# nlesc-smcm/hymls

Hardware: AMD Instinct MI355X
Metric: Preconditioner ApplyInverse DoF/s + achieved HBM GB/s, Stokes3D (higher is better)
Workload: dtype f64

## Files before the change

hymls_amd/api.py:

```python
import ctypes as C
import os
import numpy as np

LIB_PATH = os.environ.get("HYMLS_MI_LIBRARY") or os.path.join(os.path.dirname(os.path.abspath(__file__)), "libhymls_mi.so")


class HymlsError(RuntimeError):
    def __init__(self, code, msg):
        super().__init__("hymls_mi error %d: %s" % (code, msg))
        self.code = code


class _Params(C.Structure):
    _fields_ = [(n, C.c_int32) for n in (
        "nx", "ny", "nz", "dim", "equations", "dof", "sx", "sy", "sz", "cx", "cy", "cz", "levels",
        "partitioner", "retain_nodes", "retain_pressures", "link_velocities", "link_retained",
        "fix_pressure_level", "nfix")] + [("fix_gid", C.c_int32 * 4), ("variable_type", C.c_int32 * 8),
                                         ("retain_xyz", C.c_int32 * 3), ("retain_at_level", C.c_int32 * 8),
                                         ("retain_at_level_xyz", (C.c_int32 * 3) * 8), ("periodic", C.c_int32 * 3)]


_I32P = C.POINTER(C.c_int32)
_I64P = C.POINTER(C.c_int64)
_F64P = C.POINTER(C.c_double)
# ... 26 lines not shown
        "hymls_mi_default_params": (None, [C.POINTER(_Params)]),
        "hymls_mi_create": (C.c_int, [C.POINTER(H), C.POINTER(_Params), C.c_int]),
        "hymls_mi_set_matrix_csr": (C.c_int, [H, C.c_int64, _I32P, _I32P, _F64P]),
        "hymls_mi_set_comm": (C.c_int, [H, C.POINTER(_Comm), C.c_int, C.c_int, C.c_int]),
        "hymls_mi_rank_grid": (C.c_int, [C.c_int, C.POINTER(C.c_int), C.POINTER(C.c_int), C.POINTER(C.c_int)]),
        "hymls_mi_device_alloc": (C.c_void_p, [H, C.c_int64]),
        "hymls_mi_device_free": (None, [H, C.c_void_p]),
        "hymls_mi_copy_to_host": (C.c_int, [H, C.c_void_p, C.c_void_p, C.c_int64]),
        "hymls_mi_copy_to_device": (C.c_int, [H, C.c_void_p, C.c_void_p, C.c_int64]),
        "hymls_mi_rccl_unique_id": (C.c_int, [C.c_char_p]),
        "hymls_mi_rccl_comm_init": (C.c_int, [C.c_char_p, C.c_int, C.c_int, C.c_int, C.POINTER(C.c_void_p)]),
        "hymls_mi_rccl_comm_destroy": (None, [C.c_void_p]),
        "hymls_mi_set_comm_rccl": (C.c_int, [H, C.c_void_p, C.c_int, C.c_int, C.c_int]),
        "hymls_mi_comm_selftest": (C.c_int, [H]),
        "hymls_mi_invert_blocks": (C.c_int, [H, C.c_int32, C.c_int32, _F64P]),
        "hymls_mi_required_rows": (C.c_int, [H, _I64P, _I32P]),
        "hymls_mi_set_matrix_rows": (C.c_int, [H, C.c_int64, _I32P, _I32P, _I32P, _F64P]),
        "hymls_mi_owned_rows": (C.c_int, [H, _I64P, _I32P]),
        "hymls_mi_generate_rows": (C.c_int, [C.c_int, C.c_int, C.c_int, C.c_int, C.c_double, C.c_double, C.c_int64, _I32P,
                                             _I64P, _I32P, _I32P, _F64P]),
        "hymls_mi_set_testvector": (C.c_int, [H, _F64P]),
        "hymls_mi_initialize": (C.c_int, [H]),
        "hymls_mi_compute": (C.c_int, [H]),
        "hymls_mi_set_factor_storage": (C.c_int, [H, C.c_int]),
        "hymls_mi_factor_storage": (C.c_int, [H]),
        "hymls_mi_apply_inverse": (C.c_int, [H, C.c_void_p, C.c_int64, C.c_void_p, C.c_int64, C.c_int, C.c_int]),
        "hymls_mi_set_border": (C.c_int, [H, C.c_int, C.c_void_p, C.c_int64, C.c_void_p, C.c_int64, C.c_void_p]),
        "hymls_mi_apply_inverse_bordered": (C.c_int, [H, C.c_void_p, C.c_void_p, C.c_void_p, C.c_void_p, C.c_int]),
        "hymls_mi_apply": (C.c_int, [H, _F64P, _F64P]),
        "hymls_mi_matvec": (C.c_int, [H, C.c_void_p, C.c_void_p, C.c_int]),
# ... 165 lines not shown
            self.SetFactorStorage(storage)
        if comm is not None:
            comm.attach(self)
            px, py, pz = rank_grid
            if getattr(comm, "nccl_comm", None) is not None:
                self._check(self._lib.hymls_mi_set_comm_rccl(self._h, comm.nccl_comm, px, py, pz))
            else:
                self._check(self._lib.hymls_mi_set_comm(self._h, C.byref(comm.c_struct), px, py, pz))
        if K is not None:
            self.SetMatrix(K)
        if testVector is not None:
            self.SetTestVector(testVector)

    def CommSelfTest(self):
        return self._lib.hymls_mi_comm_selftest(self._h)

    def InvertBlocks(self, blocks):
        B = np.asarray(blocks, dtype=np.float64)
        assert B.ndim == 3 and B.shape[1] == B.shape[2]
        cm = np.array(B.transpose(0, 2, 1), dtype=np.float64, order="C", copy=True)
        self._check(self._lib.hymls_mi_invert_blocks(self._h, B.shape[1], B.shape[0], cm.ctypes.data_as(_F64P)))
        return np.ascontiguousarray(cm.transpose(0, 2, 1))

    def RequiredRows(self):
        n = C.c_int64()
        self._check(self._lib.hymls_mi_required_rows(self._h, C.byref(n), None))
        g = np.empty(n.value, np.int32)
        self._check(self._lib.hymls_mi_required_rows(self._h, C.byref(n), _i32(g)))
        return g

# ... 264 lines not shown
```

hymls_amd/csrc/capi.cpp:

```cpp
#include "../../include/hymls_mi.h"
#include "precond.hpp"
#include "capi_internal.hpp"
#include <chrono>
#include <cstring>

namespace hymls {
int64_t generate_laplace3d(int nx, int ny, int nz, int32_t* rowptr, int32_t* col, double* val);
int64_t generate_stokes3d(int nx, int ny, int nz, double a, double b, int32_t* rowptr, int32_t* col, double* val);
int64_t generate_rows(int equations, int nx, int ny, int nz, double a, double b, int64_t nrows, const int32_t* gids,
                      int32_t* rowptr, int32_t* col, double* val, double re, const bool* per);
}

using namespace hymls;

struct hymls_mi {
  Params p;
  int device = 0;
  dev::Context* ctx = nullptr;
  Csr K;
  bool have_matrix = false;
  Comm comm;
  ivec gids;
  int32_t nrows = 0;
  ivec rows_rowptr, rows_colgid;
// ... 231 lines not shown
    int32_t* d_flag = (int32_t*)dev::alloc(sizeof(int32_t));
    int32_t flag = 0;
    try {
      dev::h2d(d, blocks, bytes);
      dev::zero(d_flag, sizeof(int32_t));
      dev::dense_invert(nb, nblk, d, d_flag);
      dev::d2h(&flag, d_flag, sizeof flag);
      dev::d2h(blocks, d, bytes);
    } catch (...) { dev::free(d); dev::free(d_flag); throw; }
    dev::free(d); dev::free(d_flag);
    HYMLS_CHECK(flag == 0, -4, "singular block");
  }
  API_END(h)
}

int hymls_mi_required_rows(hymls_mi_t* h, int64_t* n, int32_t* gids) {
  if (!h || !n) return -2;
  API_BEGIN
  if (!h->top) { h->top.reset(new LevelSolver(h->p, 0, h->ngid(), &h->comm)); h->initialized = false; h->n_init_top = 0; }
  h->top->partition(nullptr);
  ivec r = h->top->required_gids();
  *n = (int64_t)r.size();
  if (gids) std::copy(r.begin(), r.end(), gids);
  API_END(h)
}

int hymls_mi_set_matrix_rows(hymls_mi_t* h, int64_t nrows, const int32_t* gids, const int32_t* rowptr,
                             const int32_t* colgid, const double* val) {
  if (!h || !gids || !rowptr) return -2;
  API_BEGIN
// ... 408 lines not shown
```

hymls_amd/csrc/device.hpp:

```cpp
#pragma once
#include <cstdio>
#include "common.hpp"
#include "symbolic.hpp"

namespace hymls {
namespace dev {

struct Context;
Context* create_context(int device);
void bind(Context* c);
Context* current();
void destroy_context(Context* c);
void* stream();
const double* zeros16();
void* alloc(size_t bytes);
void free(void* p);
void h2d(void* dst, const void* src, size_t bytes);
void d2h(void* dst, const void* src, size_t bytes);
void d2d(void* dst, const void* src, size_t bytes);
void zero(void* dst, size_t bytes);
void sync();
size_t mem_free();
void* shared_scratch(size_t bytes);
constexpr int NSIDE = 8;
// ... 76 lines not shown
  double* swork;
  int64_t swork_stride;
};

void gather(int64_t n, const int32_t* idx, const double* src, double* dst);
void scatter(int64_t n, const int32_t* idx, const double* src, double* dst);
void scatter_add(int64_t n, const int32_t* idx, const double* src, double* dst);
void axpby(int64_t n, double a, const double* x, double b, double* y);
void scale_copy(int64_t n, double a, const double* x, double* y);
inline int spmv_lanes(int32_t nrows, int64_t nnz_hint) {
  const double avg = nnz_hint >= 0 ? (double)nnz_hint / nrows : 8.0;
  return avg < 2.5 ? 1 : (avg < 5.0 ? 2 : (avg < 20.0 ? 4 : 8));
}
void spmv(int32_t nrows, const int32_t* rowptr, const int32_t* col, const double* val,
          const double* x, double* y, double alpha, double beta, int64_t nnz_hint = -1);
void pull_sum(int64_t n, const int64_t* ptr, const int64_t* idx, const double* in, double* out);
void offdiag_count(int64_t nrows, const int32_t* rows, const int32_t* krow, const int32_t* kcol, const int32_t* ta, const int32_t* tb,
                   const int32_t* excl, int32_t* count);
void offdiag_fill(int64_t nrows, const int32_t* rows, const int32_t* krow, const int32_t* kcol, const int32_t* ta, const int32_t* tb,
                  const int32_t* excl, const int32_t* rowptr, int32_t* col, int32_t* src);
void member_sources(int32_t nb, int32_t next, int32_t nent, const int32_t* ext, const int32_t* ent_row, const int32_t* ent_col,
                    const int32_t* krow, const int32_t* kcol, int32_t* src, int32_t* flag);
void build_pull_tables(int64_t nrows, const int64_t* rcount, const int32_t* rowptr, const uint64_t* keys, int64_t* ptr, int64_t* idx);
void pull_sum_blocks(int64_t blen, int32_t nblk, const int64_t* ptr, const int64_t* base,
                     const double* in, double* out);

void factor_level(const PlanD& P, const BatchD& B, const int32_t* list, int32_t count,
                  int32_t b0, int32_t nbc, const double* kval, int32_t max_w);
void sblock_init(const PlanD& P, const BatchD& B, int32_t b0, int32_t nbc, const double* kval);

// ... 55 lines not shown
                     const double* x, double* y);
void solve_bwd_tasks(const LvlTask* tasks, int32_t ntasks, const LvlSub* subs, const PlanD* plans, int32_t lds_doubles,
                     const double* y, double* x);

constexpr int NV_MAX = 4;
void interior_solve_fused_mv(int32_t nsub, const FusedSub* subs, const PlanD* plans, int32_t lds_doubles, int32_t front_doubles,
                             double* x, int64_t ldx, int nv);
void interior_solve_fused_mv_f32(int32_t nsub, const FusedSub* subs, const PlanD* plans, int32_t lds_doubles, int32_t front_doubles,
                                 double* x, int64_t ldx, int nv);
void solve_fwd_tasks_mv(const LvlTask* tasks, int32_t ntasks, const LvlSub* subs, const PlanD* plans, int32_t lds_doubles,
                        const double* x, double* y, int64_t ld, int nv);
void solve_bwd_tasks_mv(const LvlTask* tasks, int32_t ntasks, const LvlSub* subs, const PlanD* plans, int32_t lds_doubles,
                        const double* y, double* x, int64_t ld, int nv);

void ot_apply(int32_t ng, const int32_t* gptr, const double* w, double* x);
void sblock_transform(int32_t nS, int32_t ng, const int32_t* gptr, const double* tv,
                      double* sblock, int32_t nbc);
void sblock_extract(int32_t nS, int64_t npick, const int32_t* pick, const double* sblock,
                    double* out, int64_t out_stride, int32_t nbc);
struct KeptD {
  int32_t nS, ngl;
  const int32_t* gptr; const int32_t* glink; const int32_t* goff; const int64_t* lboff; const int32_t* lblen;
};
void sblock_kept(const KeptD& K, const double* tv, const double* sblock, double* out, int64_t out_stride, int32_t nbc);
bool sblock_kept_fits(int32_t nS, int32_t ngl);
void dense_invert(int32_t nb, int32_t nblk, double* blocks, int32_t* flag);
bool dense_invert_blocked_order(int32_t nb);
void blocks_apply(int32_t nb, int32_t nblk, const double* binv, const int32_t* ids,
                  const double* x, double* y);

// ... 11 lines not shown
```

hymls_amd/csrc/device_hip.hip:

```cpp
#include <hip/hip_runtime.h>
#include <type_traits>
#include <dlfcn.h>
#include <chrono>
#include <cstring>
#include <cfloat>
#include <array>
#include <map>
#include <string>
#include <cstdio>
#include "device.hpp"

namespace hymls {
namespace dev {

#define HIP_CHECK(call)                                                                    \
  do {                                                                                     \
    hipError_t e_ = (call);                                                                \
    if (e_ != hipSuccess)                                                                  \
      throw ::hymls::Error(-3, std::string("HIP error: ") + hipGetErrorString(e_) + " at " + \
                                   __FILE__ + ":" + std::to_string(__LINE__));             \
  } while (0)

struct MarkRec { int phase; bool begin; hipEvent_t ev; };
struct Context {
// ... 260 lines not shown
  for (int64_t i = blockIdx.x * (int64_t)blockDim.x + threadIdx.x; i < n; i += (int64_t)gridDim.x * blockDim.x) atomicAdd(&dst[idx[i]], src[i]);
}
void scatter_add(int64_t n, const int32_t* idx, const double* src, double* dst) {
  if (n <= 0) return;
  hipLaunchKernelGGL(k_scatter_add, dim3(nblocks(n, 256, 65536)), dim3(256), 0, g_stream, n, idx, src, dst); launch_check();
}
void axpby(int64_t n, double a, const double* x, double b, double* y) {
  if (n <= 0) return;
  hipLaunchKernelGGL(k_axpby, dim3(nblocks(n, 256, 8192)), dim3(256), 0, g_stream, n, a, x, b, y); launch_check();
}
void scale_copy(int64_t n, double a, const double* x, double* y) {
  if (n <= 0) return;
  hipLaunchKernelGGL(k_scale_copy, dim3(nblocks(n, 256, 8192)), dim3(256), 0, g_stream, n, a, x, y); launch_check();
}

template <int L>
__global__ void k_spmv(int32_t nrows, const int32_t* __restrict__ rp, const int32_t* __restrict__ col,
                       const double* __restrict__ val, const double* __restrict__ x, double* __restrict__ y,
                       double alpha, double beta) {
  const int lane = (int)(threadIdx.x % L);
  const int rpb = (int)blockDim.x / L;
  for (int64_t base = (int64_t)blockIdx.x * rpb; base < nrows; base += (int64_t)gridDim.x * rpb) {
    const int64_t row = base + threadIdx.x / L;
    double s = 0.0;
    if (row < nrows) {
      const int b = rp[row], e = rp[row + 1];
      for (int k = b + lane; k < e; k += L) s += val[k] * x[col[k]];
    }
#pragma unroll
    for (int off = L / 2; off > 0; off >>= 1) s += __shfl_down(s, off, L);
    if (row < nrows && lane == 0) y[row] = alpha * s + (beta == 0.0 ? 0.0 : beta * y[row]);
  }
}
void spmv(int32_t nrows, const int32_t* rp, const int32_t* col, const double* val, const double* x, double* y,
          double alpha, double beta, int64_t nnz_hint) {
  if (nrows <= 0) return;
  const int L = spmv_lanes(nrows, nnz_hint);
  const int64_t nt = (int64_t)nrows * L;
  const dim3 grid(nblocks(nt, 256));
  switch (L) {
    case 1: hipLaunchKernelGGL(k_spmv<1>, grid, dim3(256), 0, g_stream, nrows, rp, col, val, x, y, alpha, beta); break;
    case 2: hipLaunchKernelGGL(k_spmv<2>, grid, dim3(256), 0, g_stream, nrows, rp, col, val, x, y, alpha, beta); break;
    case 4: hipLaunchKernelGGL(k_spmv<4>, grid, dim3(256), 0, g_stream, nrows, rp, col, val, x, y, alpha, beta); break;
    default: hipLaunchKernelGGL(k_spmv<8>, grid, dim3(256), 0, g_stream, nrows, rp, col, val, x, y, alpha, beta); break;
  }
  launch_check();
}

__global__ void k_pull_sum(int64_t n, const int64_t* __restrict__ ptr, const int64_t* __restrict__ idx,
                           const double* __restrict__ in, double* __restrict__ out) {
  for (int64_t e = blockIdx.x * (int64_t)blockDim.x + threadIdx.x; e < n; e += (int64_t)gridDim.x * blockDim.x) {
    double s = 0.0;
    for (int64_t t = ptr[e]; t < ptr[e + 1]; t++) s += in[idx[t]];
    out[e] = s;
  }
}
void pull_sum(int64_t n, const int64_t* ptr, const int64_t* idx, const double* in, double* out) {
  if (n <= 0) return;
  hipLaunchKernelGGL(k_pull_sum, dim3(nblocks(n, 256, 65536)), dim3(256), 0, g_stream, n, ptr, idx, in, out); launch_check();
// ... 1654 lines not shown

struct FusedFront { int32_t c0, w, ri, c_off, a_off, lf_off, idx_off, pad; int64_t lp_off, q_off; };
template <class PTR>
__device__ inline PTR lside(PTR base, int packed, int r, int w, int ri, int& c1, int& tri) {
  if (!packed) { c1 = w + ri; tri = 0; return base + r; }
  if (r < w) { c1 = w; tri = 1; return base + (r - 1); }
  c1 = ri; tri = 0;
  return base + ((w * (w - 1)) >> 1) + (r - w);
}
template <class PTR>
__device__ inline PTR uside(PTR base, int packed, int i, int w, int ri, int& c1, int& tri) {
  if (!packed) { c1 = w + ri; tri = 0; return base + i; }
  c1 = 0; tri = 1;
  return base + ((w * (w - 1)) >> 1) + ri * w + i;
}
template <int L>
__device__ __forceinline__ void fused_spmv_rows(int n, int tid, gptr<int32_t> rp, gptr<int32_t> col, gptr<double> val, gptr<double> x, double* y) {
  const int lane = tid % L, rpb = 256 / L;
  for (int base = 0; base < n; base += rpb) {
    const int row = base + tid / L;
    double s = 0.0;
    if (row < n) {
      const int b = rp[row], e = rp[row + 1];
      for (int k = b + lane; k < e; k += L) s += val[k] * x[col[k]];
    }
#pragma unroll
    for (int off = L / 2; off > 0; off >>= 1) s += __shfl_down(s, off, L);
    if (row < n && lane == 0) y[row] = s + 0.0;
  }
}
template <bool PROF, class PT, int IN, int OUT>
__device__ __forceinline__ void interior_fused_body(const FusedSub* __restrict__ subs, const PlanD* __restrict__ plans,
                                                    double* __restrict__ x, long long* __restrict__ prof, const FusedIO io) {
  extern __shared__ double lds[];
  auto ldp = [](gptr<PT> q) { return (double)*q; };
  long long tp[6] = {0, 0, 0, 0, 0, 0}, t0 = 0, tstart = 0;
  auto tick = [&](int bucket) { if (PROF) { const long long t = wall_clock64(); tp[bucket] += t - t0; t0 = t; } };
  if (PROF) { t0 = wall_clock64(); tstart = t0; }
  const FusedSub S = subs[blockIdx.x];
  const PlanD P = plans[S.cls];
  double* X = lds;
  double* C = lds + P.nI;
  double* Fv = C + P.contrib_size;
// ... 808 lines not shown
    else if (!fwd) solve_bwd_tasks(tasks, ntasks, subs, plans, lds_doubles, av, bv);
    else if (v == 0) solve_fwd_tasks(tasks, ntasks, subs, plans, lds_doubles, av, bv);
    else launch_lvl_mv<1>(fwd, tasks, ntasks, subs, plans, lds_doubles, av, bv, ld, v);
    v += g;
  }
}
void solve_fwd_tasks_mv(const LvlTask* tasks, int32_t ntasks, const LvlSub* subs, const PlanD* plans, int32_t lds_doubles,
                        const double* x, double* y, int64_t ld, int nv) {
  lvl_tasks_mv(true, tasks, ntasks, subs, plans, lds_doubles, x, y, ld, nv);
}
void solve_bwd_tasks_mv(const LvlTask* tasks, int32_t ntasks, const LvlSub* subs, const PlanD* plans, int32_t lds_doubles,
                        const double* y, double* x, int64_t ld, int nv) {
  lvl_tasks_mv(false, tasks, ntasks, subs, plans, lds_doubles, y, x, ld, nv);
}

__global__ void __launch_bounds__(256) k_ot(int32_t ng, const int32_t* __restrict__ gptr, const double* __restrict__ w, double* __restrict__ x) {
  const int g = blockIdx.x * 32 + (threadIdx.x >> 3);
  const int lane = threadIdx.x & 7;
  const bool on = g < ng;
  const int b = on ? gptr[g] : 0, e = on ? gptr[g + 1] : 0;
  double s = 0.0;
  for (int i = b + lane; i < e; i += 8) s += w[i] * x[i];
#pragma unroll
  for (int off = 4; off > 0; off >>= 1) s += __shfl_xor(s, off, 64);
  for (int i = b + lane; i < e; i += 8) x[i] = 2.0 * w[i] * s - x[i];
}
void ot_apply(int32_t ng, const int32_t* gptr, const double* w, double* x) {
  if (ng <= 0) return;
  hipLaunchKernelGGL(k_ot, dim3((ng + 31) / 32), dim3(256), 0, g_stream, ng, gptr, w, x); launch_check();
}

__device__ inline bool hh_setup(const double* v, int n, double& sg, double& nrm, double& v1, double& fac1) {
  sg = v[0] < 0 ? -1.0 : (v[0] > 0 ? 1.0 : 0.0);
  double s = 0.0;
  for (int i = 0; i < n; i++) s += v[i] * v[i];
  nrm = sqrt(s) * fabs(sg);
  v1 = sg * v[0] + nrm;
  if (fabs(v1) < 1e-14 || nrm < 1e-14) return false;
  fac1 = 1.0 / (nrm * v1);
  return true;
}
template <int PASS>
__global__ void __launch_bounds__(256) k_sblock_hh(int32_t nS, int32_t ng, const int32_t* __restrict__ gptr,
                                                    const double* __restrict__ tv, double* __restrict__ sblock) {
// ... 633 lines not shown
```

hymls_amd/csrc/precond.cpp:

```cpp
#include "precond.hpp"
#include <cstring>
#include <chrono>
#include <thread>
#include <mutex>
#include <atomic>
#include <map>
#include <unordered_map>

namespace hymls {

namespace {

struct Hasher {
  uint64_t h = 1469598103934665603ULL;
  void add(const void* p, size_t n) {
    const unsigned char* c = (const unsigned char*)p;
    size_t i = 0;
    for (; i + 8 <= n; i += 8) {
      uint64_t w;
      std::memcpy(&w, c + i, 8);
      h = (h ^ w) * 0x9E3779B97F4A7C15ULL;
      h ^= h >> 29;
    }
    for (; i < n; i++) { h ^= c[i]; h *= 1099511628211ULL; }
// ... 953 lines not shown
  d_t2_ = (double*)dev::alloc((size_t)std::max(n2_ + ngs_, 1) * sizeof(double));
  d_y2_ = (double*)dev::alloc((size_t)std::max(n2_, 1) * sizeof(double));
  d_yb_ = (double*)dev::alloc((size_t)std::max(n2_, 1) * sizeof(double));
  d_a12_val_ = (double*)dev::alloc(std::max<size_t>(1, a12_col_.size()) * sizeof(double));
  d_a21_val_ = (double*)dev::alloc(std::max<size_t>(1, a21_col_.size()) * sizeof(double));
  d_flag_ = (int32_t*)dev::alloc(sizeof(int32_t));
  {
    int64_t covered = 0;
    for (size_t c = 0; c < cls_.size(); c++)
      if (cls_fused_[c]) covered += (int64_t)cls_[c]->lu.plan.nI * (int64_t)cls_[c]->lu.members.size();
    fused_io_ = n1_ > 0 && covered == n1_ && merged_.nsubs == 0 && !std::getenv("HYMLS_MI_NO_FUSED_IO");
    if (std::getenv("HYMLS_MI_VERBOSE"))
      std::fprintf(stderr, "[hymls_mi] rank %d level %d: vector passes of the apply %s the interior solve (fused classes cover %lld of %d interior rows, A12 %.2f entries per row)\n",
                   comm_->rank, level_, fused_io_ ? "fused into" : "separate from", (long long)covered, n1_, n1_ ? (double)a12_col_.size() / n1_ : 0.0);
  }
  initialized_ = true;
}

void LevelSolver::build_classes() {
  const bool verbose_bc = std::getenv("HYMLS_MI_VERBOSE") != nullptr && (level_ == 0 || std::atoi(std::getenv("HYMLS_MI_VERBOSE")) >= 2);
  double t_bc = wall();
  auto lap_bc = [&](const char* what) {
    if (!verbose_bc) return;
    std::fprintf(stderr, "[hymls_mi] rank %d level %d:   classes / %-22s %.2f s\n", comm_->rank, level_, what, wall() - t_bc);
    t_bc = wall();
  };
  const int n = K_.n;
  const int nsd = (int)hm_.sd.size();
  const int nsep = n2_ + ngs_;
  auto sidx = [&](int32_t gid) { const int l = g2l_[gid]; return l >= 0 ? pos2_[l] : -1; };
// ... 1169 lines not shown

void LevelSolver::next_apply(const double* rhs, double* sol, int64_t ld, int nv) {
  if (!comm_->distributed()) { next_->apply_inverse_mv(rhs, ld, sol, ld, nv); return; }
  const int64_t ldn = std::max<int64_t>(n_next_owned_, 1);
  for (int v = 0; v < nv; v++) xch_down_.forward(rhs + v * ld, d_nrhs_ + v * ldn);
  next_->apply_inverse_mv(d_nrhs_, ldn, d_nsol_, ldn, nv);
  for (int v = 0; v < nv; v++) {
    if (next_is_direct_) {
      if (red_.n) dev::d2d(sol + v * ld, d_nsol_ + v * ldn + glob_row_off_[comm_->rank], (size_t)red_.n * sizeof(double));
    } else {
      xch_down_.backward(d_nsol_ + v * ldn, sol + v * ld);
    }
  }
}

void LevelSolver::schur_apply(double* rhs2, int64_t ldr, double* x2, int64_t ldx, int nv) {
  dev::Range range("SchurPreconditioner", level_ + 1, "ApplyInverse");
  if (global_n2_ == 0) return;
  if (direct_schur_) {
    if (!comm_->distributed()) { next_->apply_inverse_mv(rhs2, ldr, x2, ldx, nv); return; }
    for (int v = 0; v < nv; v++) next_apply(rhs2 + v * ldr, x2 + v * ldx, 0, 1);
    return;
  }
  const int ng = (int)vs_.size();
  const int64_t ldv = std::max(ng, 1);
  for (int v = 0; v < nv; v++) dev::ot_apply(ng, d_gptr_, d_otw_, rhs2 + v * ldr);
  dev::blocks_apply_all_mv(n_blk_apply_, d_blka_, blk_max_nb_, rhs2, ldr, x2, ldx, nv);
  for (int v = 0; v < nv; v++) dev::gather(ng, d_vs_, rhs2 + v * ldr, d_vrhs_ + v * ldv);
  if (profiling && level_ == 0) dev::mark(4, true);
  next_apply(d_vrhs_, d_vsol_, ldv, nv);
  if (profiling && level_ == 0) dev::mark(4, false);
  for (int v = 0; v < nv; v++) {
    dev::scatter(ng, d_vs_, d_vsol_ + v * ldv, x2 + v * ldx);
    dev::ot_apply(ng, d_gptr_, d_otw_, x2 + v * ldx);
  }
}

void LevelSolver::apply_inverse(const double* b, double* x) { apply_inverse_mv(b, 0, x, 0, 1); }

void LevelSolver::apply_inverse_mv(const double* b, int64_t ldb, double* x, int64_t ldx, int nv) {
  dev::Range range("Preconditioner", level_ + 1, "ApplyInverse");
  HYMLS_CHECK(next_ != nullptr || global_n2_ == 0, -1, "The preconditioner has not yet been computed.");
  ensure_nvec(nv);
  const int64_t ldz = n1_ + ngi_ + n2_, ld1 = std::max(n1_, 1), ld2 = std::max(n2_ + ngs_, 1);
  double* z1 = d_z_;
  double* z2 = d_z_ + n1_ + ngi_;
  const bool fio = fused_io_ && nv == 1;
  if (profiling) dev::mark(0, true);
  for (int v = 0; v < nv; v++) {
    if (!fio) dev::gather(n1_, d_inperm_, b + v * ldb, z1 + v * ldz);
    dev::gather(n2_, d_inperm_ + n1_, b + v * ldb, z2 + v * ldz);
  }
  if (profiling) dev::mark(1, true);
  if (fio) {
    dev::FusedIO io;
    io.in = 1; io.b = b; io.perm = d_inperm_;
    interior_solve_mv(z1, ldz, 1, &io);
  } else {
    interior_solve_mv(z1, ldz, nv);
  }
  if (profiling) { dev::mark(1, false); dev::mark(2, true); }
  for (int v = 0; v < nv; v++) {
    xch_int_.forward(z1 + v * ldz, z1 + v * ldz);
    dev::spmv(n2_, d_a21_row_, d_a21_col_, d_a21_val_, z1 + v * ldz, z2 + v * ldz, -1.0, 1.0, (int64_t)a21_col_.size());
  }
  if (profiling) { dev::mark(2, false); dev::mark(3, true); }
  schur_apply(z2, ldz, d_t2_, ld2, nv);
  if (profiling) dev::mark(3, false);
  if (fio) {
    xch_sep_.forward(d_t2_, d_t2_);
    if (profiling) dev::mark(1, true);
    dev::FusedIO io;
    io.in = 2; io.a_row = d_a12_row_; io.a_col = d_a12_col_; io.a_val = d_a12_val_; io.x2 = d_t2_;
    io.a_lanes = dev::spmv_lanes(n1_, (int64_t)a12_col_.size());
    io.out = 1; io.z = z1; io.user = x; io.perm = d_inperm_;
    interior_solve_mv(d_t1_, ld1, 1, &io);
    if (profiling) dev::mark(1, false);
    dev::scatter(n2_, d_inperm_ + n1_, d_t2_, x);
    if (profiling) dev::mark(0, false);
    return;
  }
  if (profiling) dev::mark(2, true);
  for (int v = 0; v < nv; v++) {
    xch_sep_.forward(d_t2_ + v * ld2, d_t2_ + v * ld2);
    dev::spmv(n1_, d_a12_row_, d_a12_col_, d_a12_val_, d_t2_ + v * ld2, d_t1_ + v * ld1, 1.0, 0.0, (int64_t)a12_col_.size());
  }
  if (profiling) { dev::mark(2, false); dev::mark(1, true); }
  interior_solve_mv(d_t1_, ld1, nv);
  if (profiling) dev::mark(1, false);
  for (int v = 0; v < nv; v++) {
    dev::axpby(n1_, -1.0, d_t1_ + v * ld1, 1.0, z1 + v * ldz);
    dev::scatter(n1_, d_inperm_, z1 + v * ldz, x + v * ldx);
    dev::scatter(n2_, d_inperm_ + n1_, d_t2_ + v * ld2, x + v * ldx);
  }
  if (profiling) dev::mark(0, false);
}

void LevelSolver::build_matvec() {
  const int n = K_.n, nown = (int)owned_gids_.size();
  ivec user(n, -1);
  {
    int u = 0;
    for (int i = 0; i < nrows_; i++) if (intidx_[i] >= 0 || (pos2_[i] >= 0 && pos2_[i] < n2_)) user[i] = u++;
  }
  ivec row(1, 0), col, src, node(nown);
  std::vector<char> wanted(n, 0);
  ivec want;
  for (int i = 0; i < nrows_; i++) {
// ... 223 lines not shown
}

void LevelSolver::add_stats(ApplyStats& st, bool as_coarse) const {
  double f = 0, fs = 0, sp = 0, sep = 0, vec = 0;
  for (auto& cp : cls_) {
    f += 2.0 * (cp->lu.factor32 ? 4.0 : 8.0) * (double)cp->lu.plan.nnz_factor * (double)cp->lu.members.size();
    st.bytes_resident += cp->lu.resident_bytes();
    fs += 2.0 * (12.0 * (double)cp->lu.plan.nnz_sparse + 24.0 * cp->lu.plan.nI) * (double)cp->lu.members.size();
  }
  sp = 12.0 * (double)(a12_col_.size() + a21_col_.size()) + 4.0 * (n1_ + n2_ + 2);
  if (!direct_schur_) {
    sep = 2.0 * 12.0 * n2_;
    for (auto& B : blocks_) sep += (8.0 * B.nb * B.nb + 4.0 * B.nb) * B.nblk;
  }
  const double N = (double)(n1_ + n2_);
  vec = 8.0 * (4.0 * N + (fused_io_ ? 0.0 : 7.0) * n1_ + 12.0 * n2_);
  for (auto& cp : cls_) {
    st.flops_factor += (double)cp->lu.plan.flops_factor * (double)cp->lu.members.size();
    if (!direct_schur_) st.flops_transform += 4.0 * (double)cp->pat.nS * (double)cp->pat.nS * (double)cp->lu.members.size();
  }
  if (!direct_schur_) for (auto& B : blocks_) st.flops_blocks += 2.0 * (double)B.nb * B.nb * B.nb * B.nblk;
  if (as_coarse) { st.bytes_coarse += f + sp + sep + vec; st.bytes_coarse_sparse += fs + sp + sep + vec; }
  else { st.bytes_factor += f; st.bytes_factor_sparse += fs; st.bytes_spmv += sp; st.bytes_sep += sep; st.bytes_vec += vec; }
  if (next_) next_->add_stats(st, true);
}

}
```

hymls_amd/csrc/precond.hpp:

```cpp
#pragma once
#include <memory>
#include <thread>
#include <exception>
#include "common.hpp"
#include "partition.hpp"
#include "symbolic.hpp"
#include "device.hpp"
#include "comm.hpp"

namespace hymls {

struct ApplyStats {
  double bytes_factor = 0, bytes_spmv = 0, bytes_sep = 0, bytes_coarse = 0, bytes_vec = 0;
  double bytes_factor_sparse = 0, bytes_coarse_sparse = 0;
  double flops_factor = 0, flops_blocks = 0, flops_transform = 0;
  double bytes_resident = 0;
};

struct AsyncAlloc {
  std::thread th;
  void* p = nullptr;
  size_t bytes = 0;
  std::exception_ptr err;
  explicit AsyncAlloc(size_t n) : bytes(n) {
// ... 166 lines not shown
  int32_t num_rows() const { return nrows_; }
  Operator* next() const { return next_.get(); }
  LevelSolver* next_level() const { return next_level_; }
  double phase_seconds[5] = {0, 0, 0, 0, 0};
  bool profiling = false;

 private:
  struct Cls;
  struct ExtLayout { int32_t ngl = 0; std::vector<int64_t> blk_off; ivec blk_len; int64_t size = 0; };
  ExtLayout ext_layout(const Subdomain& S) const;
  void localize();
  void build_classes();
  void build_schur_setup();
  void exchange_records();
  const Csr& assemble_reduced(ivec& row_gids, dvec* tvn);
  void schur_apply(double* rhs2, int64_t ldr, double* x2, int64_t ldx, int nv);
  void next_apply(const double* rhs, double* sol, int64_t ld, int nv);
  void interior_solve_mv(double* x1, int64_t ld, int nv, const dev::FusedIO* io = nullptr);
  void ensure_nvec(int nv);
  int nvec_alloc_ = 1;
  void build_handoff(const ivec& next_owned);
  void interior_solve(double* x1);
  void interior_solve_transposed(double* x1);
  void compute_border();
  void set_next_border();
  void schur_apply_bordered(double* rhs2, const double* q, double* x2, double* S);
  void next_apply_bordered(const double* rhs, const double* T, double* sol, double* S);
  int64_t n_next_owned_ = 0;
  int bm_ = 0;
  dvec bC_, bSC_;
  double *d_bVu_ = nullptr, *d_bWu_ = nullptr;
// ... 34 lines not shown
  bool mv_ready_ = false, mv_stale_ = true;
  int32_t *d_mv_row_ = nullptr, *d_mv_col_ = nullptr, *d_mv_src_ = nullptr, *d_mv_node_ = nullptr;
  double *d_mv_val_ = nullptr, *d_mv_x_ = nullptr;
  int64_t mv_nnz_ = 0;
  void build_matvec();
  struct RecSeg { int64_t off, len; };
  std::vector<RecSeg> rec_send_;
  std::vector<int64_t> rec_scnt_, rec_rcnt_;
  int64_t rec_nsend_ = 0, rec_nrecv_ = 0, ext_recv_base_ = 0;
  bool rec_any_ = false;
  dev::FusedSub* d_fsubs_ = nullptr;
  dev::PlanD* d_fplans_ = nullptr;
  int32_t n_fsubs_ = 0, fused_lds_ = 0, fused_front_lds_ = 0, fused_vec_lds_ = 0;
  std::vector<char> cls_fused_;
  bool fused_io_ = false;
  int factor_bits_ = 64;
  int fsubs_bits_ = 64;
  void prepare_factor_storage();
  void finish_factor_storage();
  std::vector<char> cls_merged_;
  MergedSolve merged_;
  double* d_ytmp_ = nullptr;
  double* d_kval_ = nullptr;
  int32_t *d_krow_ = nullptr, *d_kcol_ = nullptr;
  int32_t* d_inperm_ = nullptr;
  double *d_z_ = nullptr, *d_t1_ = nullptr, *d_t2_ = nullptr, *d_y2_ = nullptr;
  ivec a12_row_, a21_row_;
  cvec a12_col_, a12_src_, a21_col_, a21_src_;
  int32_t *d_a12_row_ = nullptr, *d_a12_col_ = nullptr, *d_a12_src_ = nullptr;
  int32_t *d_a21_row_ = nullptr, *d_a21_col_ = nullptr, *d_a21_src_ = nullptr;
// ... 41 lines not shown
```

include/hymls_mi.h:

```cpp
#ifndef HYMLS_MI_H
#define HYMLS_MI_H

#include <stdint.h>

#ifdef __cplusplus
extern "C" {
#endif

typedef struct hymls_mi hymls_mi_t;

typedef struct hymls_mi_params {
  int32_t nx, ny, nz;
  int32_t dim;
  int32_t equations;
  int32_t dof;
  int32_t sx, sy, sz;
  int32_t cx, cy, cz;
  int32_t levels;
  int32_t partitioner;
  int32_t retain_nodes;
  int32_t retain_pressures;
  int32_t link_velocities;
  int32_t link_retained;
  int32_t fix_pressure_level;
// ... 21 lines not shown
  void* (*alloc)(void* ctx, int64_t bytes);
} hymls_mi_comm;

int hymls_mi_set_comm(hymls_mi_t* h, const hymls_mi_comm* comm, int px, int py, int pz);
int hymls_mi_rank_grid(int size, int* px, int* py, int* pz);
void* hymls_mi_device_alloc(hymls_mi_t* h, int64_t bytes);
void hymls_mi_device_free(hymls_mi_t* h, void* p);
int hymls_mi_copy_to_host(hymls_mi_t* h, void* host_dst, const void* device_src, int64_t bytes);
int hymls_mi_copy_to_device(hymls_mi_t* h, void* device_dst, const void* host_src, int64_t bytes);
int hymls_mi_rccl_unique_id(char* id128);
int hymls_mi_rccl_comm_init(const char* id128, int rank, int size, int device, void** nccl_comm);
void hymls_mi_rccl_comm_destroy(void* nccl_comm);
int hymls_mi_set_comm_rccl(hymls_mi_t* h, void* nccl_comm , int px, int py, int pz);
int hymls_mi_comm_selftest(hymls_mi_t* h);
int hymls_mi_invert_blocks(hymls_mi_t* h, int32_t nb, int32_t nblk, double* blocks);
int hymls_mi_required_rows(hymls_mi_t* h, int64_t* n, int32_t* gids);
int hymls_mi_set_matrix_rows(hymls_mi_t* h, int64_t nrows, const int32_t* gids, const int32_t* rowptr,
                             const int32_t* colgid, const double* val);
int hymls_mi_owned_rows(const hymls_mi_t* h, int64_t* n, int32_t* gids);

int hymls_mi_set_testvector(hymls_mi_t* h, const double* v);

int hymls_mi_initialize(hymls_mi_t* h);
int hymls_mi_compute(hymls_mi_t* h);

int hymls_mi_set_factor_storage(hymls_mi_t* h, int bits);
int hymls_mi_factor_storage(const hymls_mi_t* h);

int hymls_mi_apply_inverse(hymls_mi_t* h, const double* B, int64_t ldb,
                           double* X, int64_t ldx, int nvec, int on_device);
// ... 59 lines not shown
```

Baseline: 2.531 billion.

## Fuse separator gather into A21 SpMV and scatter into Householder pass

```diff
diff --git a/hymls_amd/api.py b/hymls_amd/api.py
--- a/hymls_amd/api.py
+++ b/hymls_amd/api.py
@@ -64,6 +64,8 @@
         "hymls_mi_set_comm_rccl": (C.c_int, [H, C.c_void_p, C.c_int, C.c_int, C.c_int]),
         "hymls_mi_comm_selftest": (C.c_int, [H]),
         "hymls_mi_invert_blocks": (C.c_int, [H, C.c_int32, C.c_int32, _F64P]),
+        "hymls_mi_spmv_perm_check": (C.c_int, [H, C.c_int32, C.c_int32, _I32P, _I32P, _F64P, _F64P, C.c_int64, _F64P, _I32P,
+                                              C.c_double, C.c_double, C.c_int64, _F64P, _F64P]),
         "hymls_mi_required_rows": (C.c_int, [H, _I64P, _I32P]),
         "hymls_mi_set_matrix_rows": (C.c_int, [H, C.c_int64, _I32P, _I32P, _I32P, _F64P]),
         "hymls_mi_owned_rows": (C.c_int, [H, _I64P, _I32P]),
@@ -259,6 +261,20 @@
 
     def CommSelfTest(self):
         return self._lib.hymls_mi_comm_selftest(self._h)
+
+    def SpmvPermCheck(self, rowptr, col, val, x, b, perm, alpha, beta, nnz_hint):
+        rowptr = np.ascontiguousarray(rowptr, dtype=np.int32)
+        col = np.ascontiguousarray(col, dtype=np.int32)
+        val = np.ascontiguousarray(val, dtype=np.float64)
+        x = np.ascontiguousarray(x, dtype=np.float64)
+        b = np.ascontiguousarray(b, dtype=np.float64)
+        perm = np.ascontiguousarray(perm, dtype=np.int32)
+        n = rowptr.size - 1
+        assert perm.size == n and col.size == val.size == rowptr[-1]
+        y1, y2 = np.empty(n), np.empty(n)
+        self._check(self._lib.hymls_mi_spmv_perm_check(self._h, n, x.size, _i32(rowptr), _i32(col), _f64(val), _f64(x), b.size, _f64(b),
+                                                       _i32(perm), float(alpha), float(beta), int(nnz_hint), _f64(y1), _f64(y2)))
+        return y1, y2
 
     def InvertBlocks(self, blocks):
         B = np.asarray(blocks, dtype=np.float64)
diff --git a/hymls_amd/csrc/capi.cpp b/hymls_amd/csrc/capi.cpp
--- a/hymls_amd/csrc/capi.cpp
+++ b/hymls_amd/csrc/capi.cpp
@@ -269,6 +269,46 @@
   API_END(h)
 }
 
+int hymls_mi_spmv_perm_check(hymls_mi_t* h, int32_t nrows, int32_t ncols, const int32_t* rowptr, const int32_t* col, const double* val,
+                             const double* x, int64_t nb, const double* b, const int32_t* perm, double alpha, double beta,
+                             int64_t nnz_hint, double* y_perm, double* y_ref) {
+  if (!h || nrows <= 0 || ncols <= 0 || nb <= 0 || !rowptr || !x || !b || !perm || !y_perm || !y_ref) return -2;
+  API_BEGIN
+#ifndef HYMLS_MI_FUSED_SEP
+  (void)alpha; (void)nnz_hint;
+  HYMLS_CHECK(false, -99, "this build of the device layer has no spmv_perm (HYMLS_MI_FUSED_SEP)");
+#else
+  const int64_t nnz = rowptr[nrows];
+  HYMLS_CHECK(beta != 0.0 && rowptr[0] == 0 && nnz >= 0 && (nnz == 0 || (col && val)), -2, "spmv_perm_check: bad arguments");
+  for (int32_t i = 0; i < nrows; i++) HYMLS_CHECK(rowptr[i] <= rowptr[i + 1] && perm[i] >= 0 && perm[i] < nb, -2, "spmv_perm_check: row pointer or permutation out of range");
+  for (int64_t e = 0; e < nnz; e++) HYMLS_CHECK(col[e] >= 0 && col[e] < ncols, -2, "spmv_perm_check: column out of range");
+  std::vector<void*> mem;
+  auto put = [&](const void* src, size_t bytes) {
+    void* d = dev::alloc(std::max<size_t>(bytes, 8));
+    mem.push_back(d);
+    if (src && bytes) dev::h2d(d, src, bytes);
+    return d;
+  };
+  try {
+    const int32_t* d_rp = (const int32_t*)put(rowptr, (size_t)(nrows + 1) * sizeof(int32_t));
+    const int32_t* d_col = (const int32_t*)put(col, (size_t)nnz * sizeof(int32_t));
+    const double* d_val = (const double*)put(val, (size_t)nnz * sizeof(double));
+    const double* d_x = (const double*)put(x, (size_t)ncols * sizeof(double));
+    const double* d_b = (const double*)put(b, (size_t)nb * sizeof(double));
+    const int32_t* d_perm = (const int32_t*)put(perm, (size_t)nrows * sizeof(int32_t));
+    double* d_y1 = (double*)put(nullptr, (size_t)nrows * sizeof(double));
+    double* d_y2 = (double*)put(nullptr, (size_t)nrows * sizeof(double));
+    dev::spmv_perm(nrows, d_rp, d_col, d_val, d_x, d_b, d_perm, d_y1, alpha, beta, nnz_hint);
+    dev::gather(nrows, d_perm, d_b, d_y2);
+    dev::spmv(nrows, d_rp, d_col, d_val, d_x, d_y2, alpha, beta, nnz_hint);
+    dev::d2h(y_perm, d_y1, (size_t)nrows * sizeof(double));
+    dev::d2h(y_ref, d_y2, (size_t)nrows * sizeof(double));
+  } catch (...) { for (void* q : mem) dev::free(q); throw; }
+  for (void* q : mem) dev::free(q);
+#endif
+  API_END(h)
+}
+
 int hymls_mi_required_rows(hymls_mi_t* h, int64_t* n, int32_t* gids) {
   if (!h || !n) return -2;
   API_BEGIN
diff --git a/hymls_amd/csrc/device.hpp b/hymls_amd/csrc/device.hpp
--- a/hymls_amd/csrc/device.hpp
+++ b/hymls_amd/csrc/device.hpp
@@ -114,6 +114,8 @@
 }
 void spmv(int32_t nrows, const int32_t* rowptr, const int32_t* col, const double* val,
           const double* x, double* y, double alpha, double beta, int64_t nnz_hint = -1);
+void spmv_perm(int32_t nrows, const int32_t* rowptr, const int32_t* col, const double* val, const double* x,
+               const double* b, const int32_t* perm, double* y, double alpha, double beta, int64_t nnz_hint = -1);
 void pull_sum(int64_t n, const int64_t* ptr, const int64_t* idx, const double* in, double* out);
 void offdiag_count(int64_t nrows, const int32_t* rows, const int32_t* krow, const int32_t* kcol, const int32_t* ta, const int32_t* tb,
                    const int32_t* excl, int32_t* count);
@@ -199,6 +201,7 @@
                         const double* y, double* x, int64_t ld, int nv);
 
 void ot_apply(int32_t ng, const int32_t* gptr, const double* w, double* x);
+void ot_apply_scatter(int32_t ng, const int32_t* gptr, const double* w, double* x, const int32_t* perm, double* out);
 void sblock_transform(int32_t nS, int32_t ng, const int32_t* gptr, const double* tv,
                       double* sblock, int32_t nbc);
 void sblock_extract(int32_t nS, int64_t npick, const int32_t* pick, const double* sblock,
diff --git a/hymls_amd/csrc/device_hip.hip b/hymls_amd/csrc/device_hip.hip
--- a/hymls_amd/csrc/device_hip.hip
+++ b/hymls_amd/csrc/device_hip.hip
@@ -298,10 +298,10 @@
   hipLaunchKernelGGL(k_scale_copy, dim3(nblocks(n, 256, 8192)), dim3(256), 0, g_stream, n, a, x, y); launch_check();
 }
 
-template <int L>
-__global__ void k_spmv(int32_t nrows, const int32_t* __restrict__ rp, const int32_t* __restrict__ col,
-                       const double* __restrict__ val, const double* __restrict__ x, double* __restrict__ y,
-                       double alpha, double beta) {
+template <int L, bool PERM>
+__device__ __forceinline__ void spmv_body(int32_t nrows, const int32_t* __restrict__ rp, const int32_t* __restrict__ col,
+                                          const double* __restrict__ val, const double* __restrict__ x, double* __restrict__ y,
+                                          const double* __restrict__ yin, const int32_t* __restrict__ perm, double alpha, double beta) {
   const int lane = (int)(threadIdx.x % L);
   const int rpb = (int)blockDim.x / L;
   for (int64_t base = (int64_t)blockIdx.x * rpb; base < nrows; base += (int64_t)gridDim.x * rpb) {
@@ -313,8 +313,20 @@
     }
 #pragma unroll
     for (int off = L / 2; off > 0; off >>= 1) s += __shfl_down(s, off, L);
-    if (row < nrows && lane == 0) y[row] = alpha * s + (beta == 0.0 ? 0.0 : beta * y[row]);
-  }
+    if (row < nrows && lane == 0) y[row] = alpha * s + (beta == 0.0 ? 0.0 : beta * (PERM ? yin[perm[row]] : y[row]));
+  }
+}
+template <int L>
+__global__ void k_spmv(int32_t nrows, const int32_t* __restrict__ rp, const int32_t* __restrict__ col,
+                       const double* __restrict__ val, const double* __restrict__ x, double* __restrict__ y,
+                       double alpha, double beta) {
+  spmv_body<L, false>(nrows, rp, col, val, x, y, nullptr, nullptr, alpha, beta);
+}
+template <int L>
+__global__ void k_spmv_perm(int32_t nrows, const int32_t* __restrict__ rp, const int32_t* __restrict__ col,
+                            const double* __restrict__ val, const double* __restrict__ x, double* __restrict__ y,
+                            const double* __restrict__ b, const int32_t* __restrict__ perm, double alpha, double beta) {
+  spmv_body<L, true>(nrows, rp, col, val, x, y, b, perm, alpha, beta);
 }
 void spmv(int32_t nrows, const int32_t* rp, const int32_t* col, const double* val, const double* x, double* y,
           double alpha, double beta, int64_t nnz_hint) {
@@ -327,6 +339,21 @@
     case 2: hipLaunchKernelGGL(k_spmv<2>, grid, dim3(256), 0, g_stream, nrows, rp, col, val, x, y, alpha, beta); break;
     case 4: hipLaunchKernelGGL(k_spmv<4>, grid, dim3(256), 0, g_stream, nrows, rp, col, val, x, y, alpha, beta); break;
     default: hipLaunchKernelGGL(k_spmv<8>, grid, dim3(256), 0, g_stream, nrows, rp, col, val, x, y, alpha, beta); break;
+  }
+  launch_check();
+}
+void spmv_perm(int32_t nrows, const int32_t* rp, const int32_t* col, const double* val, const double* x,
+               const double* b, const int32_t* perm, double* y, double alpha, double beta, int64_t nnz_hint) {
+  if (nrows <= 0) return;
+  HYMLS_CHECK(beta != 0.0, -2, "spmv_perm: beta = 0 reads no b; use spmv()");
+  const int L = spmv_lanes(nrows, nnz_hint);
+  const int64_t nt = (int64_t)nrows * L;
+  const dim3 grid(nblocks(nt, 256));
+  switch (L) {
+    case 1: hipLaunchKernelGGL(k_spmv_perm<1>, grid, dim3(256), 0, g_stream, nrows, rp, col, val, x, y, b, perm, alpha, beta); break;
+    case 2: hipLaunchKernelGGL(k_spmv_perm<2>, grid, dim3(256), 0, g_stream, nrows, rp, col, val, x, y, b, perm, alpha, beta); break;
+    case 4: hipLaunchKernelGGL(k_spmv_perm<4>, grid, dim3(256), 0, g_stream, nrows, rp, col, val, x, y, b, perm, alpha, beta); break;
+    default: hipLaunchKernelGGL(k_spmv_perm<8>, grid, dim3(256), 0, g_stream, nrows, rp, col, val, x, y, b, perm, alpha, beta); break;
   }
   launch_check();
 }
@@ -2011,19 +2038,54 @@
   c1 = 0; tri = 1;
   return base + ((w * (w - 1)) >> 1) + ri * w + i;
 }
+constexpr int FUSED_SPMV_BATCH = 4;
 template <int L>
 __device__ __forceinline__ void fused_spmv_rows(int n, int tid, gptr<int32_t> rp, gptr<int32_t> col, gptr<double> val, gptr<double> x, double* y) {
+  constexpr int B = FUSED_SPMV_BATCH;
   const int lane = tid % L, rpb = 256 / L;
-  for (int base = 0; base < n; base += rpb) {
-    const int row = base + tid / L;
-    double s = 0.0;
-    if (row < n) {
-      const int b = rp[row], e = rp[row + 1];
-      for (int k = b + lane; k < e; k += L) s += val[k] * x[col[k]];
-    }
-#pragma unroll
-    for (int off = L / 2; off > 0; off >>= 1) s += __shfl_down(s, off, L);
-    if (row < n && lane == 0) y[row] = s + 0.0;
+  for (int base = 0; base < n; base += B * rpb) {
+    int k[B], e[B];
+    double s[B];
+#pragma unroll
+    for (int j = 0; j < B; j++) {
+      const int row = base + j * rpb + tid / L, rc = row < n ? row : n - 1;
+      k[j] = rp[rc]; e[j] = rp[rc + 1];
+    }
+    bool more = false;
+#pragma unroll
+    for (int j = 0; j < B; j++) {
+      const bool in = base + j * rpb + tid / L < n;
+      k[j] = in ? k[j] + lane : 0; e[j] = in ? e[j] : 0; s[j] = 0.0;
+      more |= k[j] < e[j];
+    }
+    while (more) {
+      int c[B];
+      double v[B], xv[B];
+#pragma unroll
+      for (int j = 0; j < B; j++) {
+        int q = k[j] < e[j] ? k[j] : e[j] - 1;
+        q = q > 0 ? q : 0;
+        c[j] = col[q]; v[j] = val[q];
+      }
+#pragma unroll
+      for (int j = 0; j < B; j++) xv[j] = x[c[j]];
+      more = false;
+#pragma unroll
+      for (int j = 0; j < B; j++) {
+        const double t = s[j] + v[j] * xv[j];
+        s[j] = k[j] < e[j] ? t : s[j];
+        k[j] += L;
+        more |= k[j] < e[j];
+      }
+    }
+#pragma unroll
+    for (int j = 0; j < B; j++) {
+      const int row = base + j * rpb + tid / L;
+      double t = s[j];
+#pragma unroll
+      for (int off = L / 2; off > 0; off >>= 1) t += __shfl_down(t, off, L);
+      if (row < n && lane == 0) y[row] = t + 0.0;
+    }
   }
 }
 template <bool PROF, class PT, int IN, int OUT>
@@ -2862,7 +2924,9 @@
   lvl_tasks_mv(false, tasks, ntasks, subs, plans, lds_doubles, y, x, ld, nv);
 }
 
-__global__ void __launch_bounds__(256) k_ot(int32_t ng, const int32_t* __restrict__ gptr, const double* __restrict__ w, double* __restrict__ x) {
+template <bool OUT>
+__device__ __forceinline__ void ot_body(int32_t ng, const int32_t* __restrict__ gptr, const double* __restrict__ w, double* __restrict__ x,
+                                        const int32_t* __restrict__ perm, double* __restrict__ out) {
   const int g = blockIdx.x * 32 + (threadIdx.x >> 3);
   const int lane = threadIdx.x & 7;
   const bool on = g < ng;
@@ -2871,11 +2935,26 @@
   for (int i = b + lane; i < e; i += 8) s += w[i] * x[i];
 #pragma unroll
   for (int off = 4; off > 0; off >>= 1) s += __shfl_xor(s, off, 64);
-  for (int i = b + lane; i < e; i += 8) x[i] = 2.0 * w[i] * s - x[i];
+  for (int i = b + lane; i < e; i += 8) {
+    const double v = 2.0 * w[i] * s - x[i];
+    x[i] = v;
+    if (OUT) out[perm[i]] = v;
+  }
+}
+__global__ void __launch_bounds__(256) k_ot(int32_t ng, const int32_t* __restrict__ gptr, const double* __restrict__ w, double* __restrict__ x) {
+  ot_body<false>(ng, gptr, w, x, nullptr, nullptr);
+}
+__global__ void __launch_bounds__(256) k_ot_scatter(int32_t ng, const int32_t* __restrict__ gptr, const double* __restrict__ w, double* __restrict__ x,
+                                                    const int32_t* __restrict__ perm, double* __restrict__ out) {
+  ot_body<true>(ng, gptr, w, x, perm, out);
 }
 void ot_apply(int32_t ng, const int32_t* gptr, const double* w, double* x) {
   if (ng <= 0) return;
   hipLaunchKernelGGL(k_ot, dim3((ng + 31) / 32), dim3(256), 0, g_stream, ng, gptr, w, x); launch_check();
+}
+void ot_apply_scatter(int32_t ng, const int32_t* gptr, const double* w, double* x, const int32_t* perm, double* out) {
+  if (ng <= 0) return;
+  hipLaunchKernelGGL(k_ot_scatter, dim3((ng + 31) / 32), dim3(256), 0, g_stream, ng, gptr, w, x, perm, out); launch_check();
 }
 
 __device__ inline bool hh_setup(const double* v, int n, double& sg, double& nrm, double& v1, double& fac1) {
diff --git a/hymls_amd/csrc/precond.cpp b/hymls_amd/csrc/precond.cpp
--- a/hymls_amd/csrc/precond.cpp
+++ b/hymls_amd/csrc/precond.cpp
@@ -991,6 +991,11 @@
       std::fprintf(stderr, "[hymls_mi] rank %d level %d: vector passes of the apply %s the interior solve (fused classes cover %lld of %d interior rows, A12 %.2f entries per row)\n",
                    comm_->rank, level_, fused_io_ ? "fused into" : "separate from", (long long)covered, n1_, n1_ ? (double)a12_col_.size() / n1_ : 0.0);
   }
+#ifdef HYMLS_MI_FUSED_SEP
+  fused_sep_ = n2_ > 0 && !comm_->distributed() && !std::getenv("HYMLS_MI_NO_FUSED_SEP");
+#endif
+  fused_sep_exit_ = fused_sep_ && !direct_schur_ && gptr_.size() == vs_.size() + 1 && gptr_.front() == 0 && gptr_.back() == n2_ &&
+                    std::is_sorted(gptr_.begin(), gptr_.end());
   initialized_ = true;
 }
 
@@ -2190,8 +2195,9 @@
   }
 }
 
-void LevelSolver::schur_apply(double* rhs2, int64_t ldr, double* x2, int64_t ldx, int nv) {
+void LevelSolver::schur_apply(double* rhs2, int64_t ldr, double* x2, int64_t ldx, int nv, double* user) {
   dev::Range range("SchurPreconditioner", level_ + 1, "ApplyInverse");
+  HYMLS_CHECK(user == nullptr || (fused_sep_exit_ && nv == 1), -3, "the exit of x2 inside the Householder pass needs one vector and full group coverage");
   if (global_n2_ == 0) return;
   if (direct_schur_) {
     if (!comm_->distributed()) { next_->apply_inverse_mv(rhs2, ldr, x2, ldx, nv); return; }
@@ -2208,6 +2214,10 @@
   if (profiling && level_ == 0) dev::mark(4, false);
   for (int v = 0; v < nv; v++) {
     dev::scatter(ng, d_vs_, d_vsol_ + v * ldv, x2 + v * ldx);
+#ifdef HYMLS_MI_FUSED_SEP
+    if (user) dev::ot_apply_scatter(ng, d_gptr_, d_otw_, x2, d_inperm_ + n1_, user);
+    else
+#endif
     dev::ot_apply(ng, d_gptr_, d_otw_, x2 + v * ldx);
   }
 }
@@ -2222,10 +2232,11 @@
   double* z1 = d_z_;
   double* z2 = d_z_ + n1_ + ngi_;
   const bool fio = fused_io_ && nv == 1;
+  const bool fsep = fused_sep_ && nv == 1, fexit = fused_sep_exit_ && nv == 1;
   if (profiling) dev::mark(0, true);
   for (int v = 0; v < nv; v++) {
     if (!fio) dev::gather(n1_, d_inperm_, b + v * ldb, z1 + v * ldz);
-    dev::gather(n2_, d_inperm_ + n1_, b + v * ldb, z2 + v * ldz);
+    if (!fsep) dev::gather(n2_, d_inperm_ + n1_, b + v * ldb, z2 + v * ldz);
   }
   if (profiling) dev::mark(1, true);
   if (fio) {
@@ -2238,10 +2249,14 @@
   if (profiling) { dev::mark(1, false); dev::mark(2, true); }
   for (int v = 0; v < nv; v++) {
     xch_int_.forward(z1 + v * ldz, z1 + v * ldz);
+#ifdef HYMLS_MI_FUSED_SEP
+    if (fsep) dev::spmv_perm(n2_, d_a21_row_, d_a21_col_, d_a21_val_, z1, b, d_inperm_ + n1_, z2, -1.0, 1.0, (int64_t)a21_col_.size());
+    else
+#endif
     dev::spmv(n2_, d_a21_row_, d_a21_col_, d_a21_val_, z1 + v * ldz, z2 + v * ldz, -1.0, 1.0, (int64_t)a21_col_.size());
   }
   if (profiling) { dev::mark(2, false); dev::mark(3, true); }
-  schur_apply(z2, ldz, d_t2_, ld2, nv);
+  schur_apply(z2, ldz, d_t2_, ld2, nv, fexit ? x : nullptr);
   if (profiling) dev::mark(3, false);
   if (fio) {
     xch_sep_.forward(d_t2_, d_t2_);
@@ -2252,7 +2267,7 @@
     io.out = 1; io.z = z1; io.user = x; io.perm = d_inperm_;
     interior_solve_mv(d_t1_, ld1, 1, &io);
     if (profiling) dev::mark(1, false);
-    dev::scatter(n2_, d_inperm_ + n1_, d_t2_, x);
+    if (!fexit) dev::scatter(n2_, d_inperm_ + n1_, d_t2_, x);
     if (profiling) dev::mark(0, false);
     return;
   }
@@ -2267,7 +2282,7 @@
   for (int v = 0; v < nv; v++) {
     dev::axpby(n1_, -1.0, d_t1_ + v * ld1, 1.0, z1 + v * ldz);
     dev::scatter(n1_, d_inperm_, z1 + v * ldz, x + v * ldx);
-    dev::scatter(n2_, d_inperm_ + n1_, d_t2_ + v * ld2, x + v * ldx);
+    if (!fexit) dev::scatter(n2_, d_inperm_ + n1_, d_t2_ + v * ld2, x + v * ldx);
   }
   if (profiling) dev::mark(0, false);
 }
@@ -2521,7 +2536,7 @@
     for (auto& B : blocks_) sep += (8.0 * B.nb * B.nb + 4.0 * B.nb) * B.nblk;
   }
   const double N = (double)(n1_ + n2_);
-  vec = 8.0 * (4.0 * N + (fused_io_ ? 0.0 : 7.0) * n1_ + 12.0 * n2_);
+  vec = 8.0 * (4.0 * N + (fused_io_ ? 0.0 : 7.0) * n1_ + (12.0 - (fused_sep_ ? 2.0 : 0.0) - (fused_sep_exit_ ? 1.0 : 0.0)) * n2_);
   for (auto& cp : cls_) {
     st.flops_factor += (double)cp->lu.plan.flops_factor * (double)cp->lu.members.size();
     if (!direct_schur_) st.flops_transform += 4.0 * (double)cp->pat.nS * (double)cp->pat.nS * (double)cp->lu.members.size();
diff --git a/hymls_amd/csrc/precond.hpp b/hymls_amd/csrc/precond.hpp
--- a/hymls_amd/csrc/precond.hpp
+++ b/hymls_amd/csrc/precond.hpp
@@ -204,7 +204,7 @@
   void build_schur_setup();
   void exchange_records();
   const Csr& assemble_reduced(ivec& row_gids, dvec* tvn);
-  void schur_apply(double* rhs2, int64_t ldr, double* x2, int64_t ldx, int nv);
+  void schur_apply(double* rhs2, int64_t ldr, double* x2, int64_t ldx, int nv, double* user = nullptr);
   void next_apply(const double* rhs, double* sol, int64_t ld, int nv);
   void interior_solve_mv(double* x1, int64_t ld, int nv, const dev::FusedIO* io = nullptr);
   void ensure_nvec(int nv);
@@ -269,6 +269,7 @@
   int32_t n_fsubs_ = 0, fused_lds_ = 0, fused_front_lds_ = 0, fused_vec_lds_ = 0;
   std::vector<char> cls_fused_;
   bool fused_io_ = false;
+  bool fused_sep_ = false, fused_sep_exit_ = false;
   int factor_bits_ = 64;
   int fsubs_bits_ = 64;
   void prepare_factor_storage();
diff --git a/include/hymls_mi.h b/include/hymls_mi.h
--- a/include/hymls_mi.h
+++ b/include/hymls_mi.h
@@ -59,6 +59,9 @@
 int hymls_mi_set_comm_rccl(hymls_mi_t* h, void* nccl_comm , int px, int py, int pz);
 int hymls_mi_comm_selftest(hymls_mi_t* h);
 int hymls_mi_invert_blocks(hymls_mi_t* h, int32_t nb, int32_t nblk, double* blocks);
+int hymls_mi_spmv_perm_check(hymls_mi_t* h, int32_t nrows, int32_t ncols, const int32_t* rowptr, const int32_t* col, const double* val,
+                             const double* x, int64_t nb, const double* b, const int32_t* perm, double alpha, double beta,
+                             int64_t nnz_hint, double* y_perm, double* y_ref);
 int hymls_mi_required_rows(hymls_mi_t* h, int64_t* n, int32_t* gids);
 int hymls_mi_set_matrix_rows(hymls_mi_t* h, int64_t nrows, const int32_t* gids, const int32_t* rowptr,
                              const int32_t* colgid, const double* val);
```

Result: slower. 2.472 billion (-2.3%).
